# fabiojbg/LLMApiGateway

Hardware: AMD Instinct MI355X
Metric: req/sec @ fixed QPS (higher is better)
Workload: dtype bf16; 1 GPU; model=llama-3-8b, global_batch=256, seq_len=192, prompt_len=128, parallelism=dp1, mode=open-loop-poisson, sampling=greedy, kv_dtype=auto

## Files before the change

### llmapigateway_amd/ops/__init__.py

```python

from __future__ import annotations

import os
from typing import Optional, Tuple

_TUNE_BASE = os.path.join(os.path.dirname(os.path.abspath(__file__)), "tunableop_gfx950.csv")
if os.path.exists(_TUNE_BASE.replace(".csv", "0.csv")):
    os.environ.setdefault("PYTORCH_TUNABLEOP_ENABLED", "1")
    os.environ.setdefault("PYTORCH_TUNABLEOP_TUNING", "0")
    os.environ.setdefault("PYTORCH_TUNABLEOP_FILENAME", _TUNE_BASE)

import torch

if torch.version.hip and os.path.exists(_TUNE_BASE.replace(".csv", "0.csv")):
    try:
        import torch.cuda.tunable as _tunable

        _tunable.enable(True)
        if os.environ.get("PYTORCH_TUNABLEOP_TUNING") != "1":
            _tunable.tuning_enable(False)
            _tunable.set_filename(_TUNE_BASE, insert_device_ordinal=True)
            _tunable.read_file(_TUNE_BASE.replace(".csv", "0.csv"))
    except Exception:
        pass

from . import reference
from .reference import build_rope_cache
from .reference import (
    fp8_dequantize_weight,
    fp8_quantize_weight,
    swizzle_weight_frag_fp8,
    unswizzle_weight_frag_fp8,
)
from .reference import (
    mxfp4_dequantize_weight,
    mxfp4_quantize_weight,
    swizzle_weight_frag_mxfp4,
    unswizzle_weight_frag_mxfp4,
)

_C = None
_C_ERR: Optional[str] = None
try:
    import importlib

    _C = importlib.import_module("._C", __name__)
except ImportError as e:
    _C_ERR = str(e)


def have_native() -> bool:
    return _C is not None


def _native():
    if _C is None:
        raise RuntimeError(
            "llmapigateway_amd.ops._C (gfx950 HIP extension) is not built but a GPU tensor "
            "reached the ops layer. Build it with `python setup.py build_ext --inplace` "
            f"(import error: {_C_ERR})"
        )
    return _C


def rmsnorm(x: torch.Tensor, weight: torch.Tensor, eps: float = 1e-5) -> torch.Tensor:
    if x.is_cuda:
        out = torch.empty_like(x)
        _native().rmsnorm(out, x, weight, eps)
        return out
    return reference.rmsnorm(x, weight, eps)


def rmsnorm_residual(
    x: torch.Tensor, residual: torch.Tensor, weight: torch.Tensor, eps: float = 1e-5
) -> Tuple[torch.Tensor, torch.Tensor]:
    if x.is_cuda:
        out = torch.empty_like(x)
        _native().rmsnorm_residual(out, x, residual, weight, eps)
        return out, residual
    return reference.rmsnorm_residual(x, residual, weight, eps)


def rope_inplace(
    q: torch.Tensor, k: torch.Tensor, positions: torch.Tensor, cos_sin: torch.Tensor
) -> None:
    if q.is_cuda:
        _native().rope_inplace(q, k, positions, cos_sin)
        return
    reference.rope_inplace(q, k, positions, cos_sin)


def swiglu(x: torch.Tensor) -> torch.Tensor:
    if x.is_cuda:
        inter = x.shape[-1] // 2
        out = torch.empty(
            (*x.shape[:-1], inter), dtype=x.dtype, device=x.device
        )
        _native().swiglu(out, x)
        return out
    return reference.swiglu(x)


def rope_and_kv_write(
    q: torch.Tensor,
    k: torch.Tensor,
    v: torch.Tensor,
    k_cache: torch.Tensor,
    v_cache: torch.Tensor,
    positions: torch.Tensor,
    cos_sin: torch.Tensor,
    slot_mapping: torch.Tensor,
    k_scale: Optional[torch.Tensor] = None,
    v_scale: Optional[torch.Tensor] = None,
) -> None:
    if q.is_cuda:
        _native().rope_kv_write(
            q, k, v, k_cache, v_cache, positions, cos_sin, slot_mapping,
            k_scale, v_scale,
        )
        return
    reference.rope_inplace(q, k, positions, cos_sin)
    reference.kv_cache_write(k, v, k_cache, v_cache, slot_mapping, k_scale, v_scale)


def kv_cache_write(
    k: torch.Tensor,
    v: torch.Tensor,
    k_cache: torch.Tensor,
    v_cache: torch.Tensor,
    slot_mapping: torch.Tensor,
    k_scale: Optional[torch.Tensor] = None,
    v_scale: Optional[torch.Tensor] = None,
) -> None:
    if k.is_cuda:
        _native().kv_cache_write(k, v, k_cache, v_cache, slot_mapping, k_scale, v_scale)
        return
    reference.kv_cache_write(k, v, k_cache, v_cache, slot_mapping, k_scale, v_scale)


QTILE = 64


def build_prefill_tiles(seqlens, device) -> Tuple[torch.Tensor, torch.Tensor]:
    tile_seq, tile_off = [], []
    for i, L in enumerate(seqlens):
        for off in range(0, int(L), QTILE):
            tile_seq.append(i)
            tile_off.append(off)
    return (
        torch.tensor(tile_seq, dtype=torch.int32, device=device),
        torch.tensor(tile_off, dtype=torch.int32, device=device),
    )


def attention_prefill(
    q: torch.Tensor,
    k: torch.Tensor,
    v: torch.Tensor,
    cu_seqlens: torch.Tensor,
    max_seqlen: int,
    scale: Optional[float] = None,
    causal: bool = True,
    tile_seq: Optional[torch.Tensor] = None,
    tile_off: Optional[torch.Tensor] = None,
    k_cache: Optional[torch.Tensor] = None,
    v_cache: Optional[torch.Tensor] = None,
    block_tables: Optional[torch.Tensor] = None,
    cached_lens: Optional[torch.Tensor] = None,
    k_scale: Optional[torch.Tensor] = None,
    v_scale: Optional[torch.Tensor] = None,
    window: Optional[int] = 0,
) -> torch.Tensor:
    if scale is None:
        scale = float(q.shape[-1]) ** -0.5
    window = _check_window(window)
    if q.is_cuda:
        if not causal:
            raise NotImplementedError("GPU prefill kernel is causal-only")
        if tile_seq is None or tile_off is None:
            cu = cu_seqlens.cpu().tolist()
            seqlens = [cu[i + 1] - cu[i] for i in range(len(cu) - 1)]
            tile_seq, tile_off = build_prefill_tiles(seqlens, q.device)
        out = torch.empty_like(q)
        _native().attention_prefill(
            out, q, k, v, cu_seqlens.int(), tile_seq, tile_off, float(scale),
            k_cache, v_cache, block_tables, cached_lens, k_scale, v_scale,
            window,
        )
        return out
    return reference.attention_prefill(
        q, k, v, cu_seqlens, scale, causal,
        k_cache=k_cache, v_cache=v_cache,
        block_tables=block_tables, cached_lens=cached_lens,
        k_scale=k_scale, v_scale=v_scale, window=window,
    )


def _check_window(window: Optional[int]) -> int:
    window = int(window or 0)
    if window < 0:
        raise ValueError(f"window must be >= 0, got {window}")
    return window


_SPLIT_SPAN = 2048
_DECODE_VER = int(os.environ.get("LLMAPI_DECODE_VER", "2"))


class _Scratch:

    def __init__(self, dtype: torch.dtype):
        self.dtype = dtype
        self.bufs: dict = {}
        self.retired: list = []

    def get(self, device, numel: int) -> torch.Tensor:
        device = torch.device(device)
        buf = self.bufs.get(device.index)
        if buf is None or buf.numel() < numel:
            if buf is not None:
                self.retired.append(buf)
            buf = torch.empty(numel, dtype=self.dtype, device=device)
            self.bufs[device.index] = buf
        return buf


_decode_acc = _Scratch(torch.float32)
_decode_ml = _Scratch(torch.float32)
_slabs = _Scratch(torch.float32)
_w8_dq = _Scratch(torch.bfloat16)


def attention_decode(
    q: torch.Tensor,
    k_cache: torch.Tensor,
    v_cache: torch.Tensor,
    block_tables: torch.Tensor,
    context_lens: torch.Tensor,
    scale: Optional[float] = None,
    k_scale: Optional[torch.Tensor] = None,
    v_scale: Optional[torch.Tensor] = None,
    window: Optional[int] = 0,
) -> torch.Tensor:
    if scale is None:
        scale = float(q.shape[-1]) ** -0.5
    window = _check_window(window)
    if q.is_cuda:
        out = torch.empty_like(q)
        B, Hq = q.shape[0], q.shape[1]
        max_ctx = block_tables.shape[1] * k_cache.shape[2]
        if window:
            max_ctx = min(max_ctx, window + 64)
        nsplit = 1
        if B * k_cache.shape[1] < 192 and max_ctx > _SPLIT_SPAN:
            nsplit = min(8, -(-max_ctx // _SPLIT_SPAN))
        if nsplit > 1:
            pa = _decode_acc.get(q.device, B * Hq * nsplit * q.shape[2])
            pm = _decode_ml.get(q.device, B * Hq * nsplit * 2)
            _native().attention_decode(
                out, q, k_cache, v_cache, block_tables, context_lens,
                float(scale), pa, pm, nsplit, k_scale, v_scale, 1, window,
            )
        else:
            _native().attention_decode(
                out, q, k_cache, v_cache, block_tables, context_lens,
                float(scale), None, None, 1, k_scale, v_scale, _DECODE_VER,
                window,
            )
        return out
    return reference.attention_decode(
        q, k_cache, v_cache, block_tables, context_lens, scale,
        k_scale=k_scale, v_scale=v_scale, window=window,
    )


_SKINNY_MAX_M = int(os.environ.get("SKINNY_GEMM_MAX_M", "16"))
_SKINNY_MAX_N = 28672


def _stream_nsk(N: int, K: int, kstep: int) -> int:
    tiles = N // 64
    nsk = max(1, -(-256 // tiles))
    return min(nsk, max(1, (K // kstep) // 8), 8)


def _skinny_nsk(N: int, K: int) -> int:
    return _stream_nsk(N, K, 32)


def _w8_nsk(N: int, K: int) -> int:
    return _stream_nsk(N, K, 64)


def _w4_nsk(N: int, K: int) -> int:
    return _stream_nsk(N, K, 64)


def _gemm_skinny(x: torch.Tensor, w: torch.Tensor, swizzled: bool) -> torch.Tensor:
    M, K = x.shape
    N = w.shape[1] if swizzled else w.shape[0]
    y = torch.empty((M, N), dtype=torch.bfloat16, device=x.device)
    nsk = _skinny_nsk(N, K)
    ws = _slabs.get(x.device, nsk * M * N) if nsk > 1 else None
    _native().gemm_skinny(y, x, w, ws, nsk, swizzled)
    return y


def _splitk_norm(launch, x: torch.Tensor, N: int, nsk: int, residual, norm_w, eps):
    M = x.shape[0]
    out = torch.empty((M, N), dtype=torch.bfloat16, device=x.device)
    ws = _slabs.get(x.device, nsk * M * N)
    launch(out, ws, residual, norm_w, float(eps), out)
    return out, residual


def swizzle_weight(w: torch.Tensor) -> torch.Tensor:
    N, K = w.shape
    assert K % 32 == 0 and N % 64 == 0
    return w.view(N, K // 32, 32).permute(1, 0, 2).contiguous()


def swizzle_weight_frag(w: torch.Tensor) -> torch.Tensor:
    N, K = w.shape
    assert K % 64 == 0 and N % 64 == 0
    return (
        w.view(N // 16, 16, K // 32, 4, 8)
        .permute(2, 0, 3, 1, 4)
        .reshape(K // 32, N // 16, 64, 8)
        .contiguous()
    )


def _m256_config(M: int, N: int, K: int) -> Optional[dict]:
    if M > 256:
        return None
    if N == 8192 and K % 64 == 0 and K >= 8192:
        if K > 8192:
            return {"nf": 8, "nsk": 4, "variant": 1, "pipe": 0}
        return {"nf": 8, "nsk": 4, "variant": 0, "pipe": 0}
    if N == 7168 and K <= 8192:
        return {"nf": 4, "nsk": 3, "variant": 0, "pipe": 4}
    if N > 4096:
        return None
    if K > 8192 and N % 128 == 0:
        return {"nf": 8, "nsk": 8, "variant": 0, "pipe": 0}
    if N < 2048:
        return None
    if K < 2048:
        return {"nf": 4, "nsk": 1, "variant": 1, "pipe": 0}
    tiles = N // 64
    nsk = max(1, min(-(-256 // tiles), (K // 64) // 2, 8))
    return {"nf": 4, "nsk": nsk, "variant": 0, "pipe": 4}


def _m256_nsk(N: int, K: int, nf: int) -> int:
    tiles = N // (16 * nf)
    if tiles >= 256:
        return 1
    nsk = -(-256 // tiles)
    return max(1, min(nsk, (K // 64) // 2, 8))


_SKINNY_SWZ_MAX_M = int(os.environ.get("SKINNY_GEMM_SWZ_MAX_M", "256"))


_M256_VARIANT = int(os.environ.get("LLMAPI_M256_VARIANT", "0"))


def gemm_m256(
    x: torch.Tensor, w_frag: torch.Tensor, nf: Optional[int] = None,
    nsk: Optional[int] = None, variant: Optional[int] = None,
    pipe: Optional[int] = None,
) -> torch.Tensor:
    M, K = x.shape
    N = w_frag.shape[1] * 16
    if nf is None:
        if N % 128 == 0 and M > 64:
            nf = 8
        else:
            nf = 8 if N // 64 >= 448 else 4
    if N % (16 * nf) != 0:
        nf = 4
    if nsk is None:
        nsk = _m256_nsk(N, K, nf)
    if variant is None:
        variant = _M256_VARIANT
    if pipe is None:
        pipe = 3 if (variant == 0 and nf == 8 and K % 32 == 0) else 0
    if variant == 0:
        if pipe in (2, 3) and nf != 8:
            pipe = 0
        if pipe in (1, 4, 5) and nf != 4:
            pipe = 0
    y = torch.empty((M, N), dtype=torch.bfloat16, device=x.device)
    ws = _slabs.get(x.device, nsk * M * N) if nsk > 1 else None
    _native().gemm_m256(y, x, w_frag, ws, nsk, nf, variant, pipe, 0)
    return y


def _reduce_norm_covers(N: int) -> bool:
    return N % 512 == 0 and 0 < N <= 8192


def gemm_m256_rmsnorm_residual(
    x: torch.Tensor, w_frag: torch.Tensor, residual: torch.Tensor,
    norm_w: torch.Tensor, eps: float, nf: int, nsk: int, variant: int = 0,
    pipe: int = 0,
) -> Tuple[torch.Tensor, torch.Tensor]:
    if nsk < 2:
        raise ValueError("fused reduce+norm needs split-K slabs (nsk > 1)")
    return _splitk_norm(
        lambda y, ws, *tail: _native().gemm_m256(
            y, x, w_frag, ws, nsk, nf, variant, pipe, 0, *tail
        ),
        x, w_frag.shape[1] * 16, nsk, residual, norm_w, eps,
    )


def _linear_route(
    M: int, N: int, K: int, twin: Optional[str], eligible: bool = True
) -> Tuple[str, dict]:
    if not (
        eligible
        and M > 0
        and N % 64 == 0
        and N <= _SKINNY_MAX_N
        and K % 32 == 0
    ):
        return "library", {}
    if twin == "frag" and 8 < M <= 256 and K % 64 == 0:
        cfg = _m256_config(M, N, K)
        return ("m256", cfg) if cfg is not None else ("library", {})
    if twin == "kmajor" and M <= _SKINNY_SWZ_MAX_M:
        return "skinny", {"swizzled": True}
    if M <= _SKINNY_MAX_M:
        return "skinny", {"swizzled": False}
    return "library", {}


def _route_of(
    x: torch.Tensor, w: torch.Tensor, w_swz: Optional[torch.Tensor]
) -> Tuple[str, dict]:
    twin = None if w_swz is None else {4: "frag", 3: "kmajor"}.get(w_swz.dim())
    eligible = (
        x.is_cuda
        and x.dim() == 2
        and x.dtype == torch.bfloat16
        and w.dtype == torch.bfloat16
        and x.is_contiguous()
        and w.is_contiguous()
    )
    return _linear_route(x.shape[0], w.shape[0], w.shape[1], twin, eligible)


def linear_rmsnorm_residual(
    x: torch.Tensor, w: torch.Tensor, w_swz: Optional[torch.Tensor],
    residual: torch.Tensor, norm_w: torch.Tensor, eps: float = 1e-5,
) -> Tuple[torch.Tensor, torch.Tensor]:
    if not x.is_cuda:
        return reference.linear_rmsnorm_residual(x, w, residual, norm_w, eps)
    if not os.environ.get("LLMAPI_NO_DECODE_FUSION"):
        route, cfg = _route_of(x, w, w_swz)
        if (
            route == "m256"
            and cfg["nsk"] > 1
            and _reduce_norm_covers(w.shape[0])
            and residual.is_contiguous()
        ):
            return gemm_m256_rmsnorm_residual(
                x, w_swz, residual, norm_w, eps, **cfg
            )
    return rmsnorm_residual(linear(x, w, w_swz), residual, norm_w, eps)


def interleave_gate_up(w: torch.Tensor) -> torch.Tensor:
    two_i, K = w.shape
    assert two_i % 32 == 0
    return w.view(2, two_i // 32, 16, K).transpose(0, 1).reshape(two_i, K)


def gemm_m256_swiglu(
    x: torch.Tensor, w_frag: torch.Tensor, nf: int = 8, variant: int = 1,
    pipe: int = 0,
) -> torch.Tensor:
    M, K = x.shape
    N = w_frag.shape[1] * 16
    y = torch.empty((M, N // 2), dtype=torch.bfloat16, device=x.device)
    _native().gemm_m256(y, x, w_frag, None, 1, nf, variant, pipe, 1)
    return y


def _m256_swiglu_config(M: int, N: int, K: int) -> Optional[dict]:
    if os.environ.get("LLMAPI_NO_FUSED_SWIGLU"):
        return None
    if not (8 < M <= 256):
        return None
    if N == 28672 and K == 4096:
        if M <= 128:
            return {"nf": 8, "variant": 0, "pipe": 0}
        return {"nf": 8, "variant": 1, "pipe": 0}
    if N == 7168 and K == 4096:
        return {"nf": 4, "variant": 0, "pipe": 4}
    return None


def swiglu_linear(
    x: torch.Tensor, w: torch.Tensor,
    w_swz: Optional[torch.Tensor] = None,
    w_int: Optional[torch.Tensor] = None,
) -> torch.Tensor:
    if w_int is not None and x.dim() == 2:
        cfg = _m256_swiglu_config(x.shape[0], w_int.shape[1] * 16, x.shape[1])
        if cfg is not None:
            return gemm_m256_swiglu(x, w_int, **cfg)
    return swiglu(linear(x, w, w_swz))


def linear(
    x: torch.Tensor, w: torch.Tensor, w_swz: Optional[torch.Tensor] = None
) -> torch.Tensor:
    route, kw = _route_of(x, w, w_swz)
    if route == "m256":
        return gemm_m256(x, w_swz, **kw)
    if route == "skinny":
        return _gemm_skinny(x, w_swz if kw["swizzled"] else w, kw["swizzled"])
    return torch.nn.functional.linear(x, w)


_W8_MAX_M = 256


def w8_reserve_dequant(device, numel: int) -> torch.Tensor:
    return _w8_dq.get(device, numel)


def dequant_w8(
    q_frag: torch.Tensor, scale: torch.Tensor, out: Optional[torch.Tensor] = None
) -> torch.Tensor:
    K, N = q_frag.shape[0] * 64, q_frag.shape[1] * 16
    if not q_frag.is_cuda:
        w = reference.fp8_dequantize_weight(
            reference.unswizzle_weight_frag_fp8(q_frag), scale, torch.bfloat16
        )
        if out is not None:
            out.copy_(w)
            return out
        return w
    if out is None:
        out = w8_reserve_dequant(q_frag.device, N * K)[: N * K].view(N, K)
    _native().dequant_w8(out, q_frag, scale)
    return out


def _w8_gpu_check(x: torch.Tensor) -> None:
    if x.dim() != 2 or x.dtype != torch.bfloat16 or not x.is_contiguous():
        raise RuntimeError(
            "linear_w8 / linear_w4 on GPU need a contiguous 2-D bf16 activation "
            f"(got dim={x.dim()}, dtype={x.dtype}, contiguous={x.is_contiguous()})"
        )


def _w8_m256_default(M: int, N: int, K: int) -> dict:
    if N % 128 == 0 and M > 64:
        nf = 8
    else:
        nf = 8 if N // 64 >= 448 else 4
    if N % (16 * nf) != 0:
        nf = 4
    return {"nf": nf, "nsk": _m256_nsk(N, K, nf)}


_W8_M256_TABLE = {
    (6144, 4096): {
        64: (4, 8),
        128: (4, 8),
        256: (8, 4),
    },
    (4096, 4096): {
        64: None,
        128: (4, 8),
        256: (4, 4),
    },
    (28672, 4096): {
        64: (4, 2),
        128: (8, 2),
        256: (8, 1),
    },
    (4096, 14336): {
        64: None,
        128: (4, 8),
        256: (8, 8),
    },
    (10240, 8192): {
        64: (8, 8),
        128: (4, 4),
        256: (8, 2),
    },
    (8192, 8192): {
        64: (4, 8),
        128: (8, 8),
        256: (8, 4),
    },
    (57344, 8192): {
        64: (4, 1),
        128: (8, 1),
        256: (8, 1),
    },
    (8192, 28672): {
        64: (4, 8),
        128: (8, 8),
        256: (8, 4),
    },
}
_W8_M256_MS = (64, 128, 256)


def _w8_m256_config(M: int, N: int, K: int) -> Optional[dict]:
    row = _W8_M256_TABLE.get((N, K))
    if row is None or not (_W8_M256_MS[0] <= M <= _W8_M256_MS[-1]):
        return None
    hi = next(i for i, m in enumerate(_W8_M256_MS) if m >= M)
    cell = row[_W8_M256_MS[hi]]
    if cell is None or (M != _W8_M256_MS[hi] and row[_W8_M256_MS[hi - 1]] is None):
        return None
    return {"nf": cell[0], "nsk": cell[1]}


def _w8_macro_config(M: int, N: int, K: int) -> Optional[dict]:
    knob = os.environ.get("LLMAPI_W8_MACRO_MIN_M")
    if not knob or not (int(knob) <= M <= _W8_MAX_M):
        return None
    return _w8_m256_config(M, N, K)


def gemm_w8_m256(
    x: torch.Tensor, q_frag: torch.Tensor, scale: torch.Tensor,
    nf: Optional[int] = None, nsk: Optional[int] = None,
) -> torch.Tensor:
    M, K = x.shape
    N = q_frag.shape[1] * 16
    cfg = _w8_m256_default(M, N, K)
    if nf is None:
        nf = cfg["nf"]
    if nsk is None:
        nsk = cfg["nsk"] if nf == cfg["nf"] else _m256_nsk(N, K, nf)
    y = torch.empty((M, N), dtype=torch.bfloat16, device=x.device)
    ws = _slabs.get(x.device, nsk * M * N) if nsk > 1 else None
    _native().gemm_w8_m256(y, x, q_frag, scale, ws, nsk, nf)
    return y


def gemm_w8_m256_rmsnorm_residual(
    x: torch.Tensor, q_frag: torch.Tensor, scale: torch.Tensor,
    residual: torch.Tensor, norm_w: torch.Tensor, eps: float, nf: int,
    nsk: int,
) -> Tuple[torch.Tensor, torch.Tensor]:
    if nsk < 2:
        raise ValueError("fused reduce+norm needs split-K slabs (nsk > 1)")
    return _splitk_norm(
        lambda y, ws, *tail: _native().gemm_w8_m256(
            y, x, q_frag, scale, ws, nsk, nf, *tail
        ),
        x, q_frag.shape[1] * 16, nsk, residual, norm_w, eps,
    )


def linear_w8(
    x: torch.Tensor, q_frag: torch.Tensor, scale: torch.Tensor,
    nsk: Optional[int] = None,
) -> torch.Tensor:
    if not x.is_cuda:
        return reference.linear_w8(
            x, reference.unswizzle_weight_frag_fp8(q_frag), scale
        )
    _w8_gpu_check(x)
    M, K = x.shape
    N = q_frag.shape[1] * 16
    if M > _W8_MAX_M:
        return torch.nn.functional.linear(x, dequant_w8(q_frag, scale))
    if nsk is None:
        macro = _w8_macro_config(M, N, K)
        if macro is not None:
            return gemm_w8_m256(x, q_frag, scale, **macro)
        nsk = _w8_nsk(N, K)
    y = torch.empty((M, N), dtype=torch.bfloat16, device=x.device)
    ws = _slabs.get(x.device, nsk * M * N) if nsk > 1 else None
    _native().gemm_w8(y, x, q_frag, scale, ws, nsk)
    return y


def linear_w8_rmsnorm_residual(
    x: torch.Tensor, q_frag: torch.Tensor, scale: torch.Tensor,
    residual: torch.Tensor, norm_w: torch.Tensor, eps: float = 1e-5,
    nsk: Optional[int] = None,
) -> Tuple[torch.Tensor, torch.Tensor]:
    if x.is_cuda and not os.environ.get("LLMAPI_NO_DECODE_FUSION"):
        _w8_gpu_check(x)
        M, K = x.shape
        N = q_frag.shape[1] * 16
        macro = _w8_macro_config(M, N, K) if nsk is None else None
        if macro is not None:
            if (
                macro["nsk"] > 1
                and _reduce_norm_covers(N)
                and residual.is_contiguous()
            ):
                return gemm_w8_m256_rmsnorm_residual(
                    x, q_frag, scale, residual, norm_w, eps, **macro
                )
            return rmsnorm_residual(
                gemm_w8_m256(x, q_frag, scale, **macro), residual, norm_w, eps
            )
        k = _w8_nsk(N, K) if nsk is None else nsk
        if (
            M <= _W8_MAX_M
            and k > 1
            and _reduce_norm_covers(N)
            and residual.is_contiguous()
        ):
            return _splitk_norm(
                lambda y, ws, *tail: _native().gemm_w8(
                    y, x, q_frag, scale, ws, k, *tail
                ),
                x, N, k, residual, norm_w, eps,
            )
    return rmsnorm_residual(linear_w8(x, q_frag, scale, nsk), residual, norm_w, eps)



def dequant_w4(
    q_frag: torch.Tensor, s_frag: torch.Tensor, out: Optional[torch.Tensor] = None
) -> torch.Tensor:
    K, N = q_frag.shape[0] * 64, q_frag.shape[1] * 16
    if not q_frag.is_cuda:
        w = reference.mxfp4_dequantize_weight(
            *reference.unswizzle_weight_frag_mxfp4(q_frag, s_frag), torch.bfloat16
        )
        if out is not None:
            out.copy_(w)
            return out
        return w
    if out is None:
        out = w8_reserve_dequant(q_frag.device, N * K)[: N * K].view(N, K)
    _native().dequant_w4(out, q_frag, s_frag)
    return out


def _w4_m256_default(M: int, N: int, K: int) -> dict:
    return _w8_m256_default(M, N, K)


_W4_M256_TABLE = {
    (6144, 4096): {
        64: (4, 8),
        128: (8, 8),
        256: (8, 4),
    },
    (4096, 4096): {
        64: None,
        128: (4, 4),
        256: (4, 4),
    },
    (28672, 4096): {
        64: (4, 2),
        128: (4, 1),
        256: (8, 1),
    },
    (4096, 14336): {
        64: None,
        128: (4, 8),
        256: (8, 8),
    },
    (10240, 8192): {
        64: (8, 8),
        128: (4, 4),
        256: (4, 4),
    },
    (8192, 8192): {
        64: (4, 8),
        128: (8, 8),
        256: (8, 4),
    },
    (57344, 8192): {
        64: (4, 1),
        128: (8, 1),
        256: (8, 1),
    },
    (8192, 28672): {
        64: (4, 8),
        128: (8, 8),
        256: (8, 4),
    },
}
_W4_M256_MS = (64, 128, 256)


def _w4_m256_config(M: int, N: int, K: int) -> Optional[dict]:
    row = _W4_M256_TABLE.get((N, K))
    if row is None or not (_W4_M256_MS[0] <= M <= _W4_M256_MS[-1]):
        return None
    hi = next(i for i, m in enumerate(_W4_M256_MS) if m >= M)
    cell = row[_W4_M256_MS[hi]]
    if cell is None or (M != _W4_M256_MS[hi] and row[_W4_M256_MS[hi - 1]] is None):
        return None
    return {"nf": cell[0], "nsk": cell[1]}


def _w4_macro_config(M: int, N: int, K: int) -> Optional[dict]:
    knob = os.environ.get("LLMAPI_W4_MACRO_MIN_M")
    if not knob or not (int(knob) <= M <= _W8_MAX_M):
        return None
    return _w4_m256_config(M, N, K)


def gemm_w4_m256(
    x: torch.Tensor, q_frag: torch.Tensor, s_frag: torch.Tensor,
    nf: Optional[int] = None, nsk: Optional[int] = None,
) -> torch.Tensor:
    M, K = x.shape
    N = q_frag.shape[1] * 16
    cfg = _w4_m256_default(M, N, K)
    if nf is None:
        nf = cfg["nf"]
    if nsk is None:
        nsk = cfg["nsk"] if nf == cfg["nf"] else _m256_nsk(N, K, nf)
    y = torch.empty((M, N), dtype=torch.bfloat16, device=x.device)
    ws = _slabs.get(x.device, nsk * M * N) if nsk > 1 else None
    _native().gemm_w4_m256(y, x, q_frag, s_frag, ws, nsk, nf)
    return y


def gemm_w4_m256_rmsnorm_residual(
    x: torch.Tensor, q_frag: torch.Tensor, s_frag: torch.Tensor,
    residual: torch.Tensor, norm_w: torch.Tensor, eps: float, nf: int,
    nsk: int,
) -> Tuple[torch.Tensor, torch.Tensor]:
    if nsk < 2:
        raise ValueError("fused reduce+norm needs split-K slabs (nsk > 1)")
    return _splitk_norm(
        lambda y, ws, *tail: _native().gemm_w4_m256(
            y, x, q_frag, s_frag, ws, nsk, nf, *tail
        ),
        x, q_frag.shape[1] * 16, nsk, residual, norm_w, eps,
    )


def linear_w4(
    x: torch.Tensor, q_frag: torch.Tensor, s_frag: torch.Tensor,
    nsk: Optional[int] = None,
) -> torch.Tensor:
    if not x.is_cuda:
        return reference.linear_w4(
            x, *reference.unswizzle_weight_frag_mxfp4(q_frag, s_frag)
        )
    _w8_gpu_check(x)
    M, K = x.shape
    N = q_frag.shape[1] * 16
    if M > _W8_MAX_M:
        return torch.nn.functional.linear(x, dequant_w4(q_frag, s_frag))
    if nsk is None:
        macro = _w4_macro_config(M, N, K)
        if macro is not None:
            return gemm_w4_m256(x, q_frag, s_frag, **macro)
        nsk = _w4_nsk(N, K)
    y = torch.empty((M, N), dtype=torch.bfloat16, device=x.device)
    ws = _slabs.get(x.device, nsk * M * N) if nsk > 1 else None
    _native().gemm_w4(y, x, q_frag, s_frag, ws, nsk)
    return y


def linear_w4_rmsnorm_residual(
    x: torch.Tensor, q_frag: torch.Tensor, s_frag: torch.Tensor,
    residual: torch.Tensor, norm_w: torch.Tensor, eps: float = 1e-5,
    nsk: Optional[int] = None,
) -> Tuple[torch.Tensor, torch.Tensor]:
    if x.is_cuda and not os.environ.get("LLMAPI_NO_DECODE_FUSION"):
        _w8_gpu_check(x)
        M, K = x.shape
        N = q_frag.shape[1] * 16
        macro = _w4_macro_config(M, N, K) if nsk is None else None
        if macro is not None:
            if (
                macro["nsk"] > 1
                and _reduce_norm_covers(N)
                and residual.is_contiguous()
            ):
                return gemm_w4_m256_rmsnorm_residual(
                    x, q_frag, s_frag, residual, norm_w, eps, **macro
                )
            return rmsnorm_residual(
                gemm_w4_m256(x, q_frag, s_frag, **macro), residual, norm_w, eps
            )
        k = _w4_nsk(N, K) if nsk is None else nsk
        if (
            M <= _W8_MAX_M
            and k > 1
            and _reduce_norm_covers(N)
            and residual.is_contiguous()
        ):
            return _splitk_norm(
                lambda y, ws, *tail: _native().gemm_w4(
                    y, x, q_frag, s_frag, ws, k, *tail
                ),
                x, N, k, residual, norm_w, eps,
            )
    return rmsnorm_residual(linear_w4(x, q_frag, s_frag, nsk), residual, norm_w, eps)


def topk_topp_filter(
    logits: torch.Tensor, topp: torch.Tensor, topk: torch.Tensor
) -> torch.Tensor:
    if logits.is_cuda:
        _native().topk_topp_filter(logits, topp, topk)
        return logits
    return reference.topk_topp_filter(logits, topp, topk)


def sample(
    logits: torch.Tensor,
    temperature: torch.Tensor,
    noise: Optional[torch.Tensor] = None,
) -> torch.Tensor:
    if logits.is_cuda:
        out = torch.empty(logits.shape[0], dtype=torch.long, device=logits.device)
        _native().sample(out, logits, temperature, noise)
        return out
    return reference.sample(logits, temperature, noise)


__all__ = [
    "have_native",
    "build_rope_cache",
    "rmsnorm",
    "rmsnorm_residual",
    "rope_inplace",
    "rope_and_kv_write",
    "swiglu",
    "kv_cache_write",
    "linear",
    "gemm_m256",
    "gemm_m256_rmsnorm_residual",
    "linear_rmsnorm_residual",
    "swizzle_weight",
    "swizzle_weight_frag",
    "fp8_quantize_weight",
    "fp8_dequantize_weight",
    "swizzle_weight_frag_fp8",
    "unswizzle_weight_frag_fp8",
    "linear_w8",
    "linear_w8_rmsnorm_residual",
    "gemm_w8_m256",
    "gemm_w8_m256_rmsnorm_residual",
    "dequant_w8",
    "w8_reserve_dequant",
    "mxfp4_quantize_weight",
    "mxfp4_dequantize_weight",
    "swizzle_weight_frag_mxfp4",
    "unswizzle_weight_frag_mxfp4",
    "linear_w4",
    "linear_w4_rmsnorm_residual",
    "gemm_w4_m256",
    "gemm_w4_m256_rmsnorm_residual",
    "dequant_w4",
    "attention_prefill",
    "attention_decode",
    "sample",
    "topk_topp_filter",
    "reference",
]
```

### llmapigateway_amd/ops/csrc/gemm_m256.hip

```cpp

#include "common.h"
#include "gemm_launch.h"

#define GM_BK 64

typedef __attribute__((__vector_size__(8 * sizeof(short)))) short bf16x8;
typedef __attribute__((__vector_size__(4 * sizeof(float)))) float f32x4;

__device__ __forceinline__ f32x4 gm_mfma(bf16x8 a, bf16x8 b, f32x4 c) {
    return __builtin_amdgcn_mfma_f32_16x16x32_bf16(a, b, c, 0, 0, 0);
}

__device__ __forceinline__ void gm_glds16(const void* g, char* smem, int ldsoff) {
    ldsoff = __builtin_amdgcn_readfirstlane(ldsoff);
    __builtin_amdgcn_global_load_lds(
        (const __attribute__((address_space(1))) void*)g,
        (__attribute__((address_space(3))) void*)(smem + ldsoff), 16, 0, 0);
}

template <int N>
__device__ __forceinline__ void gm_vmwait() {
    asm volatile("s_waitcnt vmcnt(%0)" ::"n"(N) : "memory");
}

__device__ __forceinline__ void gm_cfence() { asm volatile("" ::: "memory"); }

__device__ __forceinline__ float gm_silu(float g) {
    return g / (1.f + __expf(-g));
}

template <int GPW, int NBUF, int A = 0>
__device__ __forceinline__ void gm_wait_ahead(int ahead) {
    if constexpr (A < NBUF) {
        if (ahead == A) gm_vmwait<A * GPW>();
        else gm_wait_ahead<GPW, NBUF, A + 1>(ahead);
    }
}

template <int MW, int NF, int BK, int NBUF, bool SPLITK, bool SWIGLU = false>
__launch_bounds__(MW * WAVE_SIZE)
__global__ void gemm_m256_kernel(
    bf16* __restrict__ y,
    float* __restrict__ yw,
    const bf16* __restrict__ x,
    const bf16* __restrict__ w,
    int M, int N, int K, int nsk) {
    static_assert(!(SWIGLU && SPLITK), "fused swiglu epilogue needs nsk=1");
    static_assert(!SWIGLU || NF % 2 == 0, "fused swiglu pairs fragments");
    constexpr int BM = MW * 32;
    constexpr int BN = NF * 16;
    constexpr int KS = BK / 32;
    constexpr int CPR = BK / 8;
    constexpr int XB = BM * BK * 2;
    constexpr int WB = BK * BN * 2;
    constexpr int BUFB = XB + WB;
    constexpr int XG_W = BK / 16;
    constexpr int WU = KS * NF;
    constexpr int WG_HI = (WU + MW - 1) / MW;
    constexpr int WG_LO = WU / MW;
    constexpr int GPW_HI = XG_W + WG_HI;
    constexpr int GPW_LO = XG_W + WG_LO;
    static_assert(NBUF * BUFB <= 160 * 1024, "LDS ring exceeds 160 KiB");

    __shared__ __attribute__((aligned(16))) char smem[NBUF * BUFB];

    const int lane = threadIdx.x & (WAVE_SIZE - 1);
    const int wave = threadIdx.x >> 6;
    const int n0 = blockIdx.x * BN;
    const int n16 = N / 16;

    const int ktiles = K / BK;
    const int kt_per = SPLITK ? (ktiles + nsk - 1) / nsk : ktiles;
    const int kt0 = SPLITK ? blockIdx.y * kt_per : 0;
    const int ntiles = min(ktiles - kt0, kt_per) > 0 ? min(ktiles - kt0, kt_per) : 0;

    const int xrow = wave * 32 + (lane / CPR);
    const int xchunk = (lane % CPR) ^ (xrow & (CPR - 1));
    const bf16* xsrc[XG_W];
#pragma unroll
    for (int i = 0; i < XG_W; ++i) {
        const int r = xrow + i * (512 / BK);
        xsrc[i] = x + (size_t)(r < M ? r : 0) * K + xchunk * 8;
    }
    const int xdst0 = wave * 32 * (BK * 2);

    int wfi[WG_HI];
#pragma unroll
    for (int j = 0; j < WG_HI; ++j) wfi[j] = wave + j * MW;
    const bool w_extra = wave < (WU % MW == 0 ? MW : WU % MW);

    f32x4 acc[2][NF];
#pragma unroll
    for (int f = 0; f < 2; ++f)
#pragma unroll
        for (int n = 0; n < NF; ++n) acc[f][n] = (f32x4){0.f, 0.f, 0.f, 0.f};

#define GM_STAGE(T)                                                            \
    do {                                                                       \
        const int kt__ = kt0 + (T);                                            \
        char* buf__ = smem + ((T) % NBUF) * BUFB;                              \
        _Pragma("unroll") for (int i = 0; i < XG_W; ++i)                       \
            gm_glds16(xsrc[i] + (size_t)(kt__)*BK, buf__,                      \
                      xdst0 + i * 1024);                                       \
        _Pragma("unroll") for (int j = 0; j < WG_HI; ++j) {                    \
            if (wfi[j] < WU) {                                                 \
                const size_t gfi__ = (size_t)(KS * kt__ + wfi[j] / NF) * n16 + \
                                     n0 / 16 + wfi[j] % NF;                    \
                gm_glds16(w + gfi__ * 512 + lane * 8, buf__,                   \
                          XB + wfi[j] * 1024);                                 \
            }                                                                  \
        }                                                                      \
    } while (0)

    const int arow0 = wave * 32 + (lane & 15);
    const int alk = lane >> 4;

    if (ntiles > 0) {
#pragma unroll
        for (int p = 0; p < NBUF - 1; ++p)
            if (p < ntiles) GM_STAGE(p);
        for (int t = 0; t < ntiles; ++t) {
            if (t + NBUF - 1 < ntiles) GM_STAGE(t + NBUF - 1);
            const int ahead = min(ntiles - 1 - t, NBUF - 1);
            if (w_extra) gm_wait_ahead<GPW_HI, NBUF>(ahead);
            else gm_wait_ahead<GPW_LO, NBUF>(ahead);
            __builtin_amdgcn_s_barrier();

            const char* buf = smem + (t % NBUF) * BUFB;
#pragma unroll
            for (int ks = 0; ks < KS; ++ks) {
                bf16x8 a[2], b[NF];
#pragma unroll
                for (int f = 0; f < 2; ++f) {
                    const int row = arow0 + f * 16;
                    const int chunk = (ks * 4 + alk) ^ (row & (CPR - 1));
                    a[f] = *(const __attribute__((address_space(3))) bf16x8*)(
                        (const __attribute__((address_space(3))) char*)buf +
                        row * (BK * 2) + chunk * 16);
                }
#pragma unroll
                for (int n = 0; n < NF; ++n)
                    b[n] = *(const __attribute__((address_space(3))) bf16x8*)(
                        (const __attribute__((address_space(3))) char*)buf +
                        XB + (ks * NF + n) * 1024 + lane * 16);
#pragma unroll
                for (int n = 0; n < NF; ++n)
#pragma unroll
                    for (int f = 0; f < 2; ++f)
                        acc[f][n] = gm_mfma(a[f], b[n], acc[f][n]);
            }
            gm_cfence();
            __builtin_amdgcn_s_barrier();
            gm_cfence();
        }
    }
#undef GM_STAGE

    const int m_base = wave * 32;
    if (SPLITK) {
        float* slab = yw + (size_t)blockIdx.y * M * N;
#pragma unroll
        for (int f = 0; f < 2; ++f)
#pragma unroll
            for (int r = 0; r < 4; ++r) {
                const int row = m_base + f * 16 + (lane >> 4) * 4 + r;
                if (row >= M) continue;
#pragma unroll
                for (int n = 0; n < NF; ++n)
                    slab[(size_t)row * N + n0 + n * 16 + (lane & 15)] =
                        acc[f][n][r];
            }
    } else if constexpr (SWIGLU) {
#pragma unroll
        for (int f = 0; f < 2; ++f)
#pragma unroll
            for (int r = 0; r < 4; ++r) {
                const int row = m_base + f * 16 + (lane >> 4) * 4 + r;
                if (row >= M) continue;
#pragma unroll
                for (int n = 0; n < NF; n += 2)
                    y[(size_t)row * (N >> 1) + (n0 >> 1) + (n >> 1) * 16 +
                      (lane & 15)] =
                        f2bf(gm_silu(acc[f][n][r]) * acc[f][n + 1][r]);
            }
    } else {
#pragma unroll
        for (int f = 0; f < 2; ++f)
#pragma unroll
            for (int r = 0; r < 4; ++r) {
                const int row = m_base + f * 16 + (lane >> 4) * 4 + r;
                if (row >= M) continue;
#pragma unroll
                for (int n = 0; n < NF; ++n)
                    y[(size_t)row * N + n0 + n * 16 + (lane & 15)] =
                        f2bf(acc[f][n][r]);
            }
    }
}


template <int MW, int NF, bool SPLITK, bool SWIGLU = false, bool NTW = false>
__launch_bounds__(MW * WAVE_SIZE)
__global__ void gemm_m256r_kernel(
    bf16* __restrict__ y, float* __restrict__ yw,
    const bf16* __restrict__ x,
    const bf16* __restrict__ w,
    int M, int N, int K, int nsk) {
    static_assert(!(SWIGLU && SPLITK), "fused swiglu epilogue needs nsk=1");
    static_assert(!SWIGLU || NF % 2 == 0, "fused swiglu pairs fragments");
    constexpr int BM = MW * 32;
    constexpr int BN = NF * 16;
    constexpr int XB = BM * GM_BK * 2;
    constexpr int WB = GM_BK * BN * 2;
    constexpr int BUFB = XB + WB;
    constexpr int XG_W = 4;
    constexpr int WG_W = (2 * NF + MW - 1) / MW;
    static_assert((2 * NF) % MW == 0, "W frag split uneven across waves");

    __shared__ __attribute__((aligned(16))) char smem[2 * BUFB];

    const int lane = threadIdx.x & (WAVE_SIZE - 1);
    const int wave = threadIdx.x >> 6;
    const int n0 = blockIdx.x * BN;
    const int n16 = N / 16;

    const int ktiles = K / GM_BK;
    const int kt_per = SPLITK ? (ktiles + nsk - 1) / nsk : ktiles;
    const int kt0 = SPLITK ? blockIdx.y * kt_per : 0;
    const int ntiles = min(ktiles - kt0, kt_per) > 0 ? min(ktiles - kt0, kt_per) : 0;

    const int xrow = wave * 32 + (lane >> 3);
    const bf16* xsrc[XG_W];
#pragma unroll
    for (int i = 0; i < XG_W; ++i) {
        const int r = xrow + i * 8;
        xsrc[i] = x + (size_t)(r < M ? r : 0) * K + (lane & 7) * 8;
    }
    const int xwoff = (xrow & (BM - 1)) * 128 + (((lane & 7) ^ (xrow & 7)) << 4);

    int wfi[WG_W];
#pragma unroll
    for (int j = 0; j < WG_W; ++j) wfi[j] = wave + j * MW;

    f32x4 acc[2][NF];
#pragma unroll
    for (int f = 0; f < 2; ++f)
#pragma unroll
        for (int n = 0; n < NF; ++n) acc[f][n] = (f32x4){0.f, 0.f, 0.f, 0.f};

    bf16x8 xr[XG_W], wr[WG_W];

#define GMR_LOAD(T)                                                            \
    do {                                                                       \
        const int kt__ = kt0 + (T);                                            \
        _Pragma("unroll") for (int i = 0; i < XG_W; ++i) xr[i] =               \
            *(const __attribute__((address_space(1))) bf16x8*)(                \
                xsrc[i] + (size_t)(kt__)*GM_BK);                               \
        _Pragma("unroll") for (int j = 0; j < WG_W; ++j) {                     \
            const size_t gfi__ = (size_t)(2 * kt__ + wfi[j] / NF) * n16 +      \
                                 n0 / 16 + wfi[j] % NF;                        \
            const __attribute__((address_space(1))) bf16x8* wp__ =             \
                (const __attribute__((address_space(1))) bf16x8*)(             \
                    w + gfi__ * 512 + lane * 8);                               \
            wr[j] = NTW ? __builtin_nontemporal_load(wp__) : *wp__;            \
        }                                                                      \
    } while (0)
#define GMR_WRITE(T)                                                           \
    do {                                                                       \
        char* buf__ = smem + ((T)&1) * BUFB;                                   \
        _Pragma("unroll") for (int i = 0; i < XG_W; ++i)                       \
            *(__attribute__((address_space(3))) bf16x8*)(                      \
                (__attribute__((address_space(3))) char*)buf__ + xwoff +       \
                i * 8 * 128) = xr[i];                                          \
        _Pragma("unroll") for (int j = 0; j < WG_W; ++j)                       \
            *(__attribute__((address_space(3))) bf16x8*)(                      \
                (__attribute__((address_space(3))) char*)buf__ + XB +          \
                wfi[j] * 1024 + lane * 16) = wr[j];                            \
    } while (0)

    const int arow0 = wave * 32 + (lane & 15);
    const int alk = lane >> 4;

    if (ntiles > 0) {
        GMR_LOAD(0);
        GMR_WRITE(0);
        if (ntiles > 1) GMR_LOAD(1);
        gm_cfence();
        __builtin_amdgcn_s_barrier();
        gm_cfence();
        for (int t = 0; t < ntiles; ++t) {
            if (t + 1 < ntiles) {
                GMR_WRITE(t + 1);
                if (t + 2 < ntiles) GMR_LOAD(t + 2);
            }
            const char* buf = smem + (t & 1) * BUFB;
#pragma unroll
            for (int ks = 0; ks < 2; ++ks) {
                bf16x8 a[2], b[NF];
#pragma unroll
                for (int f = 0; f < 2; ++f) {
                    const int row = arow0 + f * 16;
                    const int chunk = (ks * 4 + alk) ^ (row & 7);
                    a[f] = *(const __attribute__((address_space(3))) bf16x8*)(
                        (const __attribute__((address_space(3))) char*)buf +
                        (row & (BM - 1)) * 128 + chunk * 16);
                }
#pragma unroll
                for (int n = 0; n < NF; ++n)
                    b[n] = *(const __attribute__((address_space(3))) bf16x8*)(
                        (const __attribute__((address_space(3))) char*)buf +
                        XB + (ks * NF + n) * 1024 + lane * 16);
#pragma unroll
                for (int n = 0; n < NF; ++n)
#pragma unroll
                    for (int f = 0; f < 2; ++f)
                        acc[f][n] = gm_mfma(a[f], b[n], acc[f][n]);
            }
            gm_cfence();
            __builtin_amdgcn_s_barrier();
            gm_cfence();
        }
    }
#undef GMR_LOAD
#undef GMR_WRITE

    const int m_base = wave * 32;
    if (SPLITK) {
        float* slab = yw + (size_t)blockIdx.y * M * N;
#pragma unroll
        for (int f = 0; f < 2; ++f)
#pragma unroll
            for (int r = 0; r < 4; ++r) {
                const int row = m_base + f * 16 + (lane >> 4) * 4 + r;
                if (row >= M) continue;
#pragma unroll
                for (int n = 0; n < NF; ++n)
                    slab[(size_t)row * N + n0 + n * 16 + (lane & 15)] =
                        acc[f][n][r];
            }
    } else if constexpr (SWIGLU) {
#pragma unroll
        for (int f = 0; f < 2; ++f)
#pragma unroll
            for (int r = 0; r < 4; ++r) {
                const int row = m_base + f * 16 + (lane >> 4) * 4 + r;
                if (row >= M) continue;
#pragma unroll
                for (int n = 0; n < NF; n += 2)
                    y[(size_t)row * (N >> 1) + (n0 >> 1) + (n >> 1) * 16 +
                      (lane & 15)] =
                        f2bf(gm_silu(acc[f][n][r]) * acc[f][n + 1][r]);
            }
    } else {
#pragma unroll
        for (int f = 0; f < 2; ++f)
#pragma unroll
            for (int r = 0; r < 4; ++r) {
                const int row = m_base + f * 16 + (lane >> 4) * 4 + r;
                if (row >= M) continue;
#pragma unroll
                for (int n = 0; n < NF; ++n)
                    y[(size_t)row * N + n0 + n * 16 + (lane & 15)] =
                        f2bf(acc[f][n][r]);
            }
    }
}


#define PC_WAVES 8
#define PC_CONS 6
#define PC_BN (PC_CONS * 16)
#define PC_BK 64
#define PC_NSLOT 3
#define PC_WD 8

template <bool SPLITK, int ABL = 0>
__launch_bounds__(PC_WAVES * WAVE_SIZE)
__global__ void gemm_m256pc_kernel(
    bf16* __restrict__ y,
    float* __restrict__ yw,
    const bf16* __restrict__ x,
    const bf16* __restrict__ w,
    int M, int N, int K, int nsk) {
    constexpr int XB = 256 * PC_BK * 2;
    __shared__ __attribute__((aligned(16))) char smem[PC_NSLOT * XB];

    const int lane = threadIdx.x & (WAVE_SIZE - 1);
    const int wave = threadIdx.x >> 6;
    const int n0 = blockIdx.x * PC_BN;
    const int n16 = N / 16;

    const int ktiles = K / PC_BK;
    const int kt_per = SPLITK ? (ktiles + nsk - 1) / nsk : ktiles;
    const int kt0 = SPLITK ? blockIdx.y * kt_per : 0;
    const int ntiles = min(ktiles - kt0, kt_per) > 0 ? min(ktiles - kt0, kt_per) : 0;
    const int nk = ntiles * 2;

    if (wave >= PC_CONS) {
        const int lw = wave - PC_CONS;
        const int xrow = lw * 128 + (lane >> 3);
        const int xchunk = lane & 7;
        const bf16* xsrc[16];
#pragma unroll
        for (int i = 0; i < 16; ++i) {
            const int r = xrow + i * 8;
            xsrc[i] = x + (size_t)(r < M ? r : 0) * K + xchunk * 8;
        }
        const int xwoff = (xrow)*128 + ((xchunk ^ (xrow & 7)) << 4);
        bf16x8 xa[16], xb[16];
#define PC_LOAD(SET, T)                                                        \
    do {                                                                       \
        const size_t kof__ = (size_t)(kt0 + (T)) * PC_BK;                      \
        _Pragma("unroll") for (int i = 0; i < 16; ++i) SET[i] =                \
            *(const __attribute__((address_space(1))) bf16x8*)(xsrc[i] +       \
                                                               kof__);         \
    } while (0)
#define PC_WRITE(SET, T)                                                       \
    do {                                                                       \
        char* buf__ = smem + ((T) % PC_NSLOT) * XB;                            \
        _Pragma("unroll") for (int i = 0; i < 16; ++i)                         \
            *(__attribute__((address_space(3))) bf16x8*)(                      \
                (__attribute__((address_space(3))) char*)buf__ + xwoff +       \
                i * 8 * 128) = SET[i];                                         \
    } while (0)
        if (ntiles > 0) {
            if (ABL != 2) {
                PC_LOAD(xa, 0);
                PC_WRITE(xa, 0);
                if (ntiles > 1) PC_LOAD(xa, 1);
                if (ntiles > 2) PC_LOAD(xb, 2);
            }
            __syncthreads();
            for (int t = 0; t < ntiles; ++t) {
                if (ABL != 2 && t + 1 < ntiles) {
                    if (t & 1) {
                        PC_WRITE(xb, t + 1);
                        if (t + 3 < ntiles) PC_LOAD(xb, t + 3);
                    } else {
                        PC_WRITE(xa, t + 1);
                        if (t + 3 < ntiles) PC_LOAD(xa, t + 3);
                    }
                }
                __syncthreads();
            }
        }
#undef PC_LOAD
#undef PC_WRITE
        return;
    }

    const int nfrag = min(n0 / 16 + wave, n16 - 1);
    const bf16* wbase = w + (size_t)lane * 8;
    auto wsrc = [&](int ks) {
        const int g = kt0 * 2 + min(ks, nk > 0 ? nk - 1 : 0);
        return (const __attribute__((address_space(1))) bf16x8*)(
            wbase + ((size_t)g * n16 + nfrag) * 512);
    };

    f32x4 acc[16];
#pragma unroll
    for (int m = 0; m < 16; ++m) acc[m] = (f32x4){0.f, 0.f, 0.f, 0.f};

    const int arow_l = lane & 15;
    const int alk = lane >> 4;

    if (ntiles > 0 && ABL == 1) {
        __syncthreads();
        for (int t = 0; t < ntiles; ++t) __syncthreads();
    } else if (ntiles > 0) {
        bf16x8 wring[PC_WD];
#pragma unroll
        for (int d = 0; d < PC_WD; ++d) wring[d] = *wsrc(d);
        __syncthreads();

        int t = 0;
        for (; t + 4 <= ntiles && 2 * (t + 4) <= nk; t += 4) {
#pragma unroll
            for (int tt = 0; tt < 4; ++tt) {
                const char* buf = smem + ((t + tt) % PC_NSLOT) * XB;
#pragma unroll
                for (int ks = 0; ks < 2; ++ks) {
                    const int kabs = 2 * (t + tt) + ks;
                    const int ridx = kabs & (PC_WD - 1);
                    const bf16x8 bfrag = wring[ridx];
#pragma unroll
                    for (int m = 0; m < 16; ++m) {
                        const int row = m * 16 + arow_l;
                        const int chunk = (ks * 4 + alk) ^ (row & 7);
                        const bf16x8 afrag =
                            *(const __attribute__((address_space(3))) bf16x8*)(
                                (const __attribute__((address_space(3))) char*)
                                    buf +
                                row * 128 + chunk * 16);
                        acc[m] = gm_mfma(afrag, bfrag, acc[m]);
                    }
                    wring[ridx] = *wsrc(kabs + PC_WD);
                }
                __syncthreads();
            }
        }
        for (; t < ntiles; ++t) {
            const char* buf = smem + (t % PC_NSLOT) * XB;
#pragma unroll
            for (int ks = 0; ks < 2; ++ks) {
                const int kabs = 2 * t + ks;
                bf16x8 bfrag;
#pragma unroll
                for (int d = 0; d < PC_WD; ++d)
                    if (d == (kabs & (PC_WD - 1))) bfrag = wring[d];
#pragma unroll
                for (int m = 0; m < 16; ++m) {
                    const int row = m * 16 + arow_l;
                    const int chunk = (ks * 4 + alk) ^ (row & 7);
                    const bf16x8 afrag =
                        *(const __attribute__((address_space(3))) bf16x8*)(
                            (const __attribute__((address_space(3))) char*)buf +
                            row * 128 + chunk * 16);
                    acc[m] = gm_mfma(afrag, bfrag, acc[m]);
                }
            }
            __syncthreads();
        }
    }

    const int col = n0 + wave * 16 + (lane & 15);
    if (col >= N) return;
    if (SPLITK) {
        float* slab = yw + (size_t)blockIdx.y * M * N;
#pragma unroll
        for (int m = 0; m < 16; ++m)
#pragma unroll
            for (int r = 0; r < 4; ++r) {
                const int row = m * 16 + (lane >> 4) * 4 + r;
                if (row < M) slab[(size_t)row * N + col] = acc[m][r];
            }
    } else {
#pragma unroll
        for (int m = 0; m < 16; ++m)
#pragma unroll
            for (int r = 0; r < 4; ++r) {
                const int row = m * 16 + (lane >> 4) * 4 + r;
                if (row < M) y[(size_t)row * N + col] = f2bf(acc[m][r]);
            }
    }
}

extern "C" hipError_t launch_gemm_m256(
    void* y, float* workspace, const void* x, const void* w, int M, int N,
    int K, int nsk, int nf, int variant, int pipe, int swiglu,
    void* residual, const void* norm_weight, float eps, void* norm_out,
    hipStream_t stream) {
    if (M <= 0 || M > 256) return hipErrorInvalidValue;
    const bool fuse_norm = residual != nullptr;
    if (fuse_norm && (norm_weight == nullptr || norm_out == nullptr ||
                      nsk < 2 || swiglu || !gemm_reduce_rmsnorm_covers(N)))
        return hipErrorInvalidValue;
    if (nsk < 1 || (nsk > 1 && workspace == nullptr)) return hipErrorInvalidValue;
    if ((K % GM_BK) != 0) return hipErrorInvalidValue;
    if (swiglu && (nsk != 1 || variant == 2)) return hipErrorInvalidValue;
    if (variant == 2) {
        if ((N % 16) != 0) return hipErrorInvalidValue;
        dim3 grid((N + PC_BN - 1) / PC_BN, nsk);
        dim3 block(PC_WAVES * WAVE_SIZE);
#define PC_L(SPLIT)                                                                do {                                                                               if (pipe == 1)                                                                     gemm_m256pc_kernel<SPLIT, 1><<<grid, block, 0, stream>>>(                          (bf16*)y, workspace, (const bf16*)x, (const bf16*)w, M, N, K,                  nsk);                                                                  else if (pipe == 2)                                                                gemm_m256pc_kernel<SPLIT, 2><<<grid, block, 0, stream>>>(                          (bf16*)y, workspace, (const bf16*)x, (const bf16*)w, M, N, K,                  nsk);                                                                  else                                                                               gemm_m256pc_kernel<SPLIT, 0><<<grid, block, 0, stream>>>(                          (bf16*)y, workspace, (const bf16*)x, (const bf16*)w, M, N, K,                  nsk);                                                              } while (0)
        if (nsk > 1) PC_L(true);
        else PC_L(false);
#undef PC_L
        HIP_CHECK_LAST();
        return launch_splitk_tail(y, workspace, M, N, nsk, residual,
                                  norm_weight, eps, norm_out, stream);
    }
    if (nf != 4 && nf != 8) return hipErrorInvalidValue;
    if ((N % (16 * nf)) != 0) return hipErrorInvalidValue;
    if (variant == 0) {
        if ((pipe == 1 || pipe == 4 || pipe == 5) && nf != 4)
            return hipErrorInvalidValue;
        if ((pipe == 2 || pipe == 3) && nf != 8) return hipErrorInvalidValue;
    }
    int mw = 1;
    while (mw * 32 < M) mw *= 2;
    const int tiles = N / (16 * nf);
    dim3 grid(tiles, nsk);
    dim3 block(mw * WAVE_SIZE);
#define GM_L2(MWV, NFV, SPLIT, SW)                                             \
    do {                                                                       \
        if (variant == 1 && pipe == 1)                                         \
            gemm_m256r_kernel<MWV, NFV, SPLIT, SW, true><<<grid, block, 0,     \
                                                           stream>>>(         \
                (bf16*)y, workspace, (const bf16*)x, (const bf16*)w, M, N, K,  \
                nsk);                                                          \
        else if (variant == 1)                                                 \
            gemm_m256r_kernel<MWV, NFV, SPLIT, SW><<<grid, block, 0,           \
                                                     stream>>>(               \
                (bf16*)y, workspace, (const bf16*)x, (const bf16*)w, M, N, K,  \
                nsk);                                                          \
        else if (pipe == 1 && NFV == 4)                                        \
            gemm_m256_kernel<MWV, 4, 64, 4, SPLIT, SW><<<grid, block, 0,       \
                                                         stream>>>(           \
                (bf16*)y, workspace, (const bf16*)x, (const bf16*)w, M, N, K,  \
                nsk);                                                          \
        else if (pipe == 2 && NFV == 8)                                        \
            gemm_m256_kernel<MWV, 8, 32, 4, SPLIT, SW><<<grid, block, 0,       \
                                                         stream>>>(           \
                (bf16*)y, workspace, (const bf16*)x, (const bf16*)w, M, N, K,  \
                nsk);                                                          \
        else if (pipe == 3 && NFV == 8)                                        \
            gemm_m256_kernel<MWV, 8, 32, 6, SPLIT, SW><<<grid, block, 0,       \
                                                         stream>>>(           \
                (bf16*)y, workspace, (const bf16*)x, (const bf16*)w, M, N, K,  \
                nsk);                                                          \
        else if (pipe == 4 && NFV == 4)                                        \
            gemm_m256_kernel<MWV, 4, 64, 2, SPLIT, SW><<<grid, block, 0,       \
                                                         stream>>>(           \
                (bf16*)y, workspace, (const bf16*)x, (const bf16*)w, M, N, K,  \
                nsk);                                                          \
        else if (pipe == 5 && NFV == 4)                                        \
            gemm_m256_kernel<MWV, 4, 32, 3, SPLIT, SW><<<grid, block, 0,       \
                                                         stream>>>(           \
                (bf16*)y, workspace, (const bf16*)x, (const bf16*)w, M, N, K,  \
                nsk);                                                          \
        else                                                                   \
            gemm_m256_kernel<MWV, NFV, 64, 3, SPLIT, SW><<<grid, block, 0,     \
                                                           stream>>>(         \
                (bf16*)y, workspace, (const bf16*)x, (const bf16*)w, M, N, K,  \
                nsk);                                                          \
    } while (0)
#define GM_L1(MWV, NFV)                                                        \
    do {                                                                       \
        if (swiglu) GM_L2(MWV, NFV, false, true);                              \
        else if (nsk > 1) GM_L2(MWV, NFV, true, false);                        \
        else GM_L2(MWV, NFV, false, false);                                    \
    } while (0)
#define GM_L0(MWV)                                                             \
    do {                                                                       \
        if (nf == 4) GM_L1(MWV, 4);                                            \
        else GM_L1(MWV, 8);                                                    \
    } while (0)
    switch (mw) {
        case 1: GM_L0(1); break;
        case 2: GM_L0(2); break;
        case 4: GM_L0(4); break;
        default: GM_L0(8); break;
    }
#undef GM_L0
#undef GM_L1
#undef GM_L2
    HIP_CHECK_LAST();
    return launch_splitk_tail(y, workspace, M, N, nsk, residual, norm_weight,
                              eps, norm_out, stream);
}
```

Before: 187.5 req/s.

## Add two-deep register prefetch ring to m256r GEMM for fused SwiGLU

```diff
diff --git a/llmapigateway_amd/ops/__init__.py b/llmapigateway_amd/ops/__init__.py
--- a/llmapigateway_amd/ops/__init__.py
+++ b/llmapigateway_amd/ops/__init__.py
@@ -504,15 +504,25 @@
     return None
 
 
+def _m256_swiglu_ring(cfg: dict, M: int, N: int, K: int) -> dict:
+    if (
+        N == 28672 and K == 4096 and M > 64
+        and cfg["nf"] == 8 and cfg["pipe"] == 0
+    ):
+        return dict(cfg, variant=1, pipe=2)
+    return cfg
+
+
 def swiglu_linear(
     x: torch.Tensor, w: torch.Tensor,
     w_swz: Optional[torch.Tensor] = None,
     w_int: Optional[torch.Tensor] = None,
 ) -> torch.Tensor:
     if w_int is not None and x.dim() == 2:
-        cfg = _m256_swiglu_config(x.shape[0], w_int.shape[1] * 16, x.shape[1])
+        M, N, K = x.shape[0], w_int.shape[1] * 16, x.shape[1]
+        cfg = _m256_swiglu_config(M, N, K)
         if cfg is not None:
-            return gemm_m256_swiglu(x, w_int, **cfg)
+            return gemm_m256_swiglu(x, w_int, **_m256_swiglu_ring(cfg, M, N, K))
     return swiglu(linear(x, w, w_swz))
 
 
diff --git a/llmapigateway_amd/ops/csrc/gemm_m256.hip b/llmapigateway_amd/ops/csrc/gemm_m256.hip
--- a/llmapigateway_amd/ops/csrc/gemm_m256.hip
+++ b/llmapigateway_amd/ops/csrc/gemm_m256.hip
@@ -199,7 +199,8 @@
 }
 
 
-template <int MW, int NF, bool SPLITK, bool SWIGLU = false, bool NTW = false>
+template <int MW, int NF, bool SPLITK, bool SWIGLU = false, bool NTW = false,
+          int DEPTH = 1>
 __launch_bounds__(MW * WAVE_SIZE)
 __global__ void gemm_m256r_kernel(
     bf16* __restrict__ y, float* __restrict__ yw,
@@ -216,6 +217,7 @@
     constexpr int XG_W = 4;
     constexpr int WG_W = (2 * NF + MW - 1) / MW;
     static_assert((2 * NF) % MW == 0, "W frag split uneven across waves");
+    static_assert(DEPTH == 1 || DEPTH == 2, "register ring depth");
 
     __shared__ __attribute__((aligned(16))) char smem[2 * BUFB];
 
@@ -248,12 +250,12 @@
 #pragma unroll
         for (int n = 0; n < NF; ++n) acc[f][n] = (f32x4){0.f, 0.f, 0.f, 0.f};
 
-    bf16x8 xr[XG_W], wr[WG_W];
-
-#define GMR_LOAD(T)                                                            \
+    bf16x8 xr[DEPTH][XG_W], wr[DEPTH][WG_W];
+
+#define GMR_LOAD(T, S)                                                         \
     do {                                                                       \
         const int kt__ = kt0 + (T);                                            \
-        _Pragma("unroll") for (int i = 0; i < XG_W; ++i) xr[i] =               \
+        _Pragma("unroll") for (int i = 0; i < XG_W; ++i) xr[S][i] =            \
             *(const __attribute__((address_space(1))) bf16x8*)(                \
                 xsrc[i] + (size_t)(kt__)*GM_BK);                               \
         _Pragma("unroll") for (int j = 0; j < WG_W; ++j) {                     \
@@ -262,65 +264,113 @@
             const __attribute__((address_space(1))) bf16x8* wp__ =             \
                 (const __attribute__((address_space(1))) bf16x8*)(             \
                     w + gfi__ * 512 + lane * 8);                               \
-            wr[j] = NTW ? __builtin_nontemporal_load(wp__) : *wp__;            \
+            wr[S][j] = NTW ? __builtin_nontemporal_load(wp__) : *wp__;         \
         }                                                                      \
     } while (0)
-#define GMR_WRITE(T)                                                           \
+#define GMR_WRITE(T, S)                                                        \
     do {                                                                       \
         char* buf__ = smem + ((T)&1) * BUFB;                                   \
         _Pragma("unroll") for (int i = 0; i < XG_W; ++i)                       \
             *(__attribute__((address_space(3))) bf16x8*)(                      \
                 (__attribute__((address_space(3))) char*)buf__ + xwoff +       \
-                i * 8 * 128) = xr[i];                                          \
+                i * 8 * 128) = xr[S][i];                                       \
         _Pragma("unroll") for (int j = 0; j < WG_W; ++j)                       \
             *(__attribute__((address_space(3))) bf16x8*)(                      \
                 (__attribute__((address_space(3))) char*)buf__ + XB +          \
-                wfi[j] * 1024 + lane * 16) = wr[j];                            \
+                wfi[j] * 1024 + lane * 16) = wr[S][j];                         \
     } while (0)
 
     const int arow0 = wave * 32 + (lane & 15);
     const int alk = lane >> 4;
 
-    if (ntiles > 0) {
-        GMR_LOAD(0);
-        GMR_WRITE(0);
-        if (ntiles > 1) GMR_LOAD(1);
-        gm_cfence();
-        __builtin_amdgcn_s_barrier();
-        gm_cfence();
-        for (int t = 0; t < ntiles; ++t) {
-            if (t + 1 < ntiles) {
-                GMR_WRITE(t + 1);
-                if (t + 2 < ntiles) GMR_LOAD(t + 2);
-            }
-            const char* buf = smem + (t & 1) * BUFB;
-#pragma unroll
-            for (int ks = 0; ks < 2; ++ks) {
-                bf16x8 a[2], b[NF];
-#pragma unroll
-                for (int f = 0; f < 2; ++f) {
-                    const int row = arow0 + f * 16;
-                    const int chunk = (ks * 4 + alk) ^ (row & 7);
-                    a[f] = *(const __attribute__((address_space(3))) bf16x8*)(
-                        (const __attribute__((address_space(3))) char*)buf +
-                        (row & (BM - 1)) * 128 + chunk * 16);
-                }
-#pragma unroll
-                for (int n = 0; n < NF; ++n)
-                    b[n] = *(const __attribute__((address_space(3))) bf16x8*)(
-                        (const __attribute__((address_space(3))) char*)buf +
-                        XB + (ks * NF + n) * 1024 + lane * 16);
-#pragma unroll
-                for (int n = 0; n < NF; ++n)
-#pragma unroll
-                    for (int f = 0; f < 2; ++f)
-                        acc[f][n] = gm_mfma(a[f], b[n], acc[f][n]);
-            }
+#define GMR_COMPUTE(T)                                                         \
+    do {                                                                       \
+        const char* buf = smem + ((T)&1) * BUFB;                               \
+        _Pragma("unroll") for (int ks = 0; ks < 2; ++ks) {                     \
+            bf16x8 a[2], b[NF];                                                \
+            _Pragma("unroll") for (int f = 0; f < 2; ++f) {                    \
+                const int row = arow0 + f * 16;                                \
+                const int chunk = (ks * 4 + alk) ^ (row & 7);                  \
+                a[f] = *(const __attribute__((address_space(3))) bf16x8*)(     \
+                    (const __attribute__((address_space(3))) char*)buf +       \
+                    (row & (BM - 1)) * 128 + chunk * 16);                      \
+            }                                                                  \
+            _Pragma("unroll") for (int n = 0; n < NF; ++n) b[n] =              \
+                *(const __attribute__((address_space(3))) bf16x8*)(            \
+                    (const __attribute__((address_space(3))) char*)buf + XB +  \
+                    (ks * NF + n) * 1024 + lane * 16);                         \
+            _Pragma("unroll") for (int n = 0; n < NF; ++n)                     \
+                _Pragma("unroll") for (int f = 0; f < 2; ++f)                  \
+                    acc[f][n] = gm_mfma(a[f], b[n], acc[f][n]);                \
+        }                                                                      \
+        gm_cfence();                                                           \
+        __builtin_amdgcn_s_barrier();                                          \
+        gm_cfence();                                                           \
+    } while (0)
+
+    if constexpr (DEPTH == 1) {
+        if (ntiles > 0) {
+            GMR_LOAD(0, 0);
+            GMR_WRITE(0, 0);
+            if (ntiles > 1) GMR_LOAD(1, 0);
             gm_cfence();
             __builtin_amdgcn_s_barrier();
             gm_cfence();
+            for (int t = 0; t < ntiles; ++t) {
+                if (t + 1 < ntiles) {
+                    GMR_WRITE(t + 1, 0);
+                    if (t + 2 < ntiles) GMR_LOAD(t + 2, 0);
+                }
+                GMR_COMPUTE(t);
+            }
         }
-    }
+    } else {
+#define GMR_ITER(T, S)                                                         \
+    do {                                                                       \
+        if ((T) + 1 < ntiles) {                                                \
+            GMR_WRITE((T) + 1, S);                                             \
+            if ((T) + 3 < ntiles) GMR_LOAD((T) + 3, S);                        \
+        }                                                                      \
+        GMR_COMPUTE(T);                                                        \
+    } while (0)
+        if (ntiles > 0) {
+            int t = 0;
+            if (ntiles > 4) {
+                GMR_LOAD(0, 0);
+                gm_cfence();
+                GMR_LOAD(1, 1);
+                gm_cfence();
+                GMR_WRITE(0, 0);
+                GMR_LOAD(2, 0);
+                gm_cfence();
+                __builtin_amdgcn_s_barrier();
+                gm_cfence();
+                for (; t + 4 < ntiles; t += 2) {
+                    GMR_WRITE(t + 1, 1);
+                    GMR_LOAD(t + 3, 1);
+                    GMR_COMPUTE(t);
+                    GMR_WRITE(t + 2, 0);
+                    GMR_LOAD(t + 4, 0);
+                    GMR_COMPUTE(t + 1);
+                }
+            } else {
+                GMR_LOAD(0, 0);
+                if (ntiles > 1) GMR_LOAD(1, 1);
+                GMR_WRITE(0, 0);
+                if (ntiles > 2) GMR_LOAD(2, 0);
+                gm_cfence();
+                __builtin_amdgcn_s_barrier();
+                gm_cfence();
+            }
+            for (; t + 1 < ntiles; t += 2) {
+                GMR_ITER(t, 1);
+                GMR_ITER(t + 1, 0);
+            }
+            if (t < ntiles) GMR_ITER(t, 1);
+        }
+#undef GMR_ITER
+    }
+#undef GMR_COMPUTE
 #undef GMR_LOAD
 #undef GMR_WRITE
 
@@ -584,7 +634,17 @@
     dim3 block(mw * WAVE_SIZE);
 #define GM_L2(MWV, NFV, SPLIT, SW)                                             \
     do {                                                                       \
-        if (variant == 1 && pipe == 1)                                         \
+        if (variant == 1 && pipe == 3)                                         \
+            gemm_m256r_kernel<MWV, NFV, SPLIT, SW, true, 2><<<grid, block, 0,  \
+                                                              stream>>>(      \
+                (bf16*)y, workspace, (const bf16*)x, (const bf16*)w, M, N, K,  \
+                nsk);                                                          \
+        else if (variant == 1 && pipe == 2)                                    \
+            gemm_m256r_kernel<MWV, NFV, SPLIT, SW, false, 2><<<grid, block, 0, \
+                                                               stream>>>(     \
+                (bf16*)y, workspace, (const bf16*)x, (const bf16*)w, M, N, K,  \
+                nsk);                                                          \
+        else if (variant == 1 && pipe == 1)                                    \
             gemm_m256r_kernel<MWV, NFV, SPLIT, SW, true><<<grid, block, 0,     \
                                                            stream>>>(         \
                 (bf16*)y, workspace, (const bf16*)x, (const bf16*)w, M, N, K,  \
```

After: 184.8 req/s. -1.4%, worse.
